# bdaiinstitute/judo

Measured on AMD Instinct MI355X. Metric: rollouts/sec + plan-step ms, leap_cube MPPI 65536xH64, higher is better.
Workload: dtype f32

## Files before the change

### judo_amd/csrc/jh_engine_v5.hip

```cpp
#include <cstddef>
#include <type_traits>

#include "jh_coop.h"

using namespace jh_eng;
using namespace jh_coop;

namespace {

#ifdef JH_V5_WAVESTAMP
__device__ unsigned long long* g_wavestamp = nullptr;
__device__ int g_wavestamp_cap = 0;
#endif

constexpr int G = 16, RPW = 4, WAVE = 64;
constexpr int NCH = 4, NLK = 4;

constexpr int LSMAX = 16;
constexpr int WAVES_PER_EU = 2;
constexpr int WAVES_PER_BLOCK = 4;
constexpr int BFS = 33;
constexpr int PAS = 9;
constexpr int RSPAD = 4;
constexpr int C3PAD = 278;
constexpr int NSLDS = 3;
constexpr double BIGPROB = 0.999999;
constexpr int CVX_STOP_NM = 1000;
#define OPAQUE(x) asm volatile("" : "+v"(x))
#define WSYNC() do { __builtin_amdgcn_fence(__ATOMIC_RELEASE, "wavefront"); __builtin_amdgcn_wave_barrier(); __builtin_amdgcn_fence(__ATOMIC_ACQUIRE, "wavefront"); } while (0)
#ifndef JH_V5_NSLOT
#define JH_V5_NSLOT 2
#endif
#ifndef JH_V5_NSBIG
#define JH_V5_NSBIG 3
#endif
#ifndef JH_V5_CYL
#define JH_V5_CYL 0
#endif
constexpr int GCYL = 5;
constexpr int NSLOT = JH_V5_NSLOT;
constexpr int NSBIG = JH_V5_NSBIG;
constexpr int NCP = 16 * (NSBIG < NSLDS ? NSBIG : NSLDS);
constexpr int NCAP = 16 * NSBIG;
constexpr int NOVF = NCAP - NCP;
constexpr int MAXHIT = 64;
constexpr int POOL_F = 10;
constexpr int MAXG = 80, MAXLG = 8;
constexpr int CUBE = 17;
constexpr int HITPAIR = 1 << 15;
static_assert(MAXG <= 128, "hand geom pairs are packed into 14 bits");
constexpr int MAXBP = 128;
constexpr int PT_SLOT = JH_PT_SLOT, PT_MAX = JH_PT_MAX, PT_I = JH_PT_I;
constexpr int MAXBPL = 96;
constexpr int NDH = 22 * 23 / 2;
constexpr int NV = 22, NQ = 23, NU = 16, NS = 31, NS_CALTECH = 23, NX = 45, NMB = 17;
constexpr int NBC = 20;
__device__ __forceinline__ bool static_code(int b) { return b == 0 || b >= NMB; }

enum { LC_DAMP = 0, LC_KVD, LC_KP, LC_KV, LC_CLO, LC_CHI, LC_CLIM, LC_FL, LC_FB, LC_FD, LC_INVW, LC_LIMITED, LC_LO, LC_HI, LC_LK, LC_LB, LC_SI, LC_IMCK = LC_SI + 5, LC_N = 25 };

struct __attribute__((aligned(16))) RS {
  float pa[NMB][PAS];
  float xR[NMB][9];
  float qv[NV], g[NV], p[NV], ws[NV];
  float acn[6];
  float Mbb[NCH][10];
  float rhs6[6];
  float cmd[4];
  union {
    struct {
      float bs[NBC][4];
      unsigned short hits[MAXHIT];
      unsigned char bpl[MAXBPL];
    };
    struct { float pk_q[G], pk_fs[G], pk_cq[4], pk_acc; };
  };
  union {
    float pool[NCP][POOL_F];
    struct { float Hcc[21], Hbb[NCH][10], Hcb[NCH][24], Hx[6][16]; };
    struct { float Hd[NDH], dinv[NV]; };
    struct { float c3pad_[C3PAD]; float c3s[G][12]; };
  };
  int ncon, nhit;
  float pad_[RSPAD];
};

static_assert(offsetof(RS, c3s) % 16 == 0 && C3PAD >= NDH + NV && sizeof(((RS*)nullptr)->c3pad_) + sizeof(((RS*)nullptr)->c3s) <= sizeof(((RS*)nullptr)->pool), "c3 cache: aligned rows behind the Newton matrices, inside the pool's storage");
struct PoolCtx { RS* S; int* overflow; float* ovf; };

__device__ __forceinline__ void push_contact(const PoolCtx& pc, const float* pos, const float* n, float dist, int body, float mu, float tran) {
  int i = atomicAdd(&pc.S->ncon, 1);
  float* e;
  if (i < NCP) e = pc.S->pool[i];
  else if (NOVF > 0 && pc.ovf && i < NCAP) e = pc.ovf + (i - NCP) * POOL_F;
  else { if (pc.overflow) atomicAdd(pc.overflow, 1); return; }
  e[0] = pos[0]; e[1] = pos[1]; e[2] = pos[2]; e[3] = n[0]; e[4] = n[1]; e[5] = n[2]; e[6] = dist; e[7] = mu; e[8] = __int_as_float(body); e[9] = tran;
}

struct LeapSink {
  PoolCtx pc; int sides; float mu, tran; bool flip;
  __device__ __forceinline__ void push(const float* pos, const float* n, float dist) {
// ... 822 lines not shown
    if (lc[LC_LIMITED] != 0.f) {
      float dlo = q - lc[LC_LO], dhi = lc[LC_HI] - q, dist = fminf(dlo, dhi);
      if (dist < 0.f) {
        float sg = dlo < dhi ? 1.f : -1.f, imp = impedance(lc + LC_SI, dist), R = fmaxf(1e-15f, (1.f - imp) / imp * lc[LC_INVW]);
        dr.lims = sg; dr.lD = 1.f / R; dr.laref = -lc[LC_LB] * (sg * qd) - lc[LC_LK] * imp * dist;
      }
    }
    bool anyslot = false; int cmask = 0; unsigned used = 0;
#pragma unroll
    for (int k = 0; k < NS; k++) {
      anyslot |= sl[k].la >= 0;
      used |= __any(sl[k].la >= 0) ? 1u << k : 0u;
      if (HC && sl[k].la > 0 && sl[k].la != CUBE && sl[k].lb > 0 && ((sl[k].la - 1) >> 2) != ((sl[k].lb - 1) >> 2)) cmask |= 1 << (4 * ((sl[k].la - 1) >> 2) + ((sl[k].lb - 1) >> 2));
    }
    int lvl = 0, par = -1, nlev = 0; bool dense_row = false;
    if constexpr (HC) {
      cmask = gor(cmask);
      if (__any(cmask != 0)) dense_row = !chain_elim_order(cmask, c, lvl, par, nlev);
#ifdef JH_V5_COUNT
      if (l == 0 && live) {
        int dmax = 0;
        for (int a = 0; a < NCH; a++) { int d = 0; for (int b = 0; b < NCH; b++) if (b != a) d += (cmask >> (a < b ? 4 * a + b : 4 * b + a)) & 1; dmax = d > dmax ? d : dmax; }
        cnt_cls[cmask == 0 ? 0 : (dense_row ? 3 : (dmax <= 1 ? 1 : 2))]++;
      }
#endif
    }
    S.pk_q[l] = q; S.pk_fs[l] = fs_own;
    if (l == 0) { S.pk_cq[0] = qc[3]; S.pk_cq[1] = qc[4]; S.pk_cq[2] = qc[5]; S.pk_cq[3] = qc[6]; S.pk_acc = acc; }
    const float Mdiag_own = sel4(Mrow, s), iMd = 1.f / Mdiag_own;
    const float fsc_own = mck * a0c_own;
    const float snorm = gsum(fs_own * fs_own * iMd + fsc_own * fsc_own * lc[LC_IMCK]);
    const bool has_rows = gor((int)(anyslot || dr.fl > 0.f || dr.lims != 0.f)) != 0;
    iters_this = 0;
    if (!has_rows) { a_own = a0_own; ac_own = a0c_own; }
    else {
      {
        const float qws = S.ws[6 + l];
        float xl[3] = {S.ws[0], S.ws[1], S.ws[2]}, xr[3] = {S.ws[3], S.ws[4], S.ws[5]}, wa[3]; mulMV(wa, S.xR[0], xr);
        const float wsc_own = l < 3 ? S.ws[l] : (l == 3 ? wa[0] : (l == 4 ? wa[1] : (l == 5 ? wa[2] : 0.f)));
        float cs = 0.f, jx[3], jar_ws[NS][3];
#pragma unroll
        for (int k = 0; k < NS; k++) if (sl[k].la >= 0) {
          slot_Jx<HC>(sl[k], S, qc, xl, wa, S.ws, jx, V5_C3C(k));
          for (int rw = 0; rw < 3; rw++) { sl[k].jar[rw] = jx[rw] - sl[k].aref[rw]; jar_ws[k][rw] = sl[k].jar[rw]; }
          cs += cone_cost(sl[k]);
        }
        const float jf_ws = qws - dr.faref, jl_ws = dr.lims * qws - dr.laref;
        dr.jf = jf_ws; dr.jl = jl_ws;
        cs += dof_rows_cost(dr);
        float dws = qws - a0_own, md = 0.f;
#pragma unroll
        for (int j = 0; j < NLK; j++) md += Mrow[j] * (quad_get(qws, j) - quad_get(a0_own, j));
        cs += 0.5f * dws * md;
        { float dcw = wsc_own - a0c_own; cs += 0.5f * dcw * dcw * mck; }
        const float cost_ws = gsum(cs);
        S.p[6 + l] = a0_own; if (l < 6) S.p[l] = a0c_own;
        WSYNC();
        float xl0[3] = {S.p[0], S.p[1], S.p[2]}, xr0[3] = {S.p[3], S.p[4], S.p[5]};
        wa[0] = xr0[0]; wa[1] = xr0[1]; wa[2] = xr0[2];
        cs = 0.f;
#pragma unroll
        for (int k = 0; k < NS; k++) if (sl[k].la >= 0) {
          slot_Jx<HC>(sl[k], S, qc, xl0, wa, S.p, jx, V5_C3C(k));
          for (int rw = 0; rw < 3; rw++) sl[k].jar[rw] = jx[rw] - sl[k].aref[rw];
          cs += cone_cost(sl[k]);
        }
        dr.jf = a0_own - dr.faref; dr.jl = dr.lims * a0_own - dr.laref;
        cs += dof_rows_cost(dr);
        const float cost_0 = gsum(cs);
        if (cost_ws < cost_0) {
          a_own = qws; ac_own = wsc_own;
#pragma unroll
          for (int k = 0; k < NS; k++) if (sl[k].la >= 0) for (int rw = 0; rw < 3; rw++) sl[k].jar[rw] = jar_ws[k][rw];
          dr.jf = jf_ws; dr.jl = jl_ws;
        } else { a_own = a0_own; ac_own = a0c_own; }
        WSYNC();
      }
      bool act = true;
      V5_TICK(3)
      auto forget_slots = [&]() __attribute__((always_inline)) {
#pragma unroll
        for (int k = 0; k < NS; k++) { OPAQUE(sl[k].la); OPAQUE(sl[k].lb); OPAQUE(sl[k].rc[0]); OPAQUE(sl[k].rc[1]); OPAQUE(sl[k].rc[2]); }
      };
      auto newton_loop = [&](auto dense_tag) __attribute__((always_inline)) {
      constexpr bool DENSE = decltype(dense_tag)::value;
      for (int it = 0; it < cap && __any(act); it++) {
        forget_slots();
        const float da_own = a_own - a0_own, dcl = ac_own - a0c_own;
        float g_own = 0.f, hd = 0.f;
#pragma unroll
        for (int j = 0; j < NLK; j++) g_own += Mrow[j] * quad_get(da_own, j);
        {
          const float D = dr.fD, x = dr.jf, fl = dr.fl, lim = dr.fR * fl;
          const bool has = fl > 0.f, lo_ = x <= -lim, hi_ = x >= lim, mid = has & !lo_ & !hi_;
          float ga = g_own - fl, gb = g_own + fl, gm = fmaf(D, x, g_own); asm volatile("" : "+v"(ga), "+v"(gb), "+v"(gm));
          g_own = has ? (lo_ ? ga : (hi_ ? gb : gm)) : g_own;
          hd = mid ? hd + D : hd;
          const bool lon = (dr.lims != 0.f) & (dr.jl < 0.f);
          g_own = lon ? fmaf(dr.lims * dr.lD, dr.jl, g_own) : g_own;
          hd = lon ? hd + dr.lD : hd;
        }
        S.g[6 + l] = g_own;
        const bool aact0 = act && !(DENSE && dense_row);
        {
          float* hb = &S.Hbb[c][tri(s, 0)];
#pragma unroll
          for (int j = 0; j < NLK; j++) hb[j < s ? j : s] = j < s ? Mrow[j] : Mdiag_own + hd;
          for (int k = 0; k < 6; k++) S.Hcb[c][s * 6 + k] = 0.f;
          if (HC) for (int k = 0; k < 6; k++) S.Hx[0][l * 6 + k] = 0.f;
        }
        float hcp[21];
#pragma unroll
        for (int e = 0; e < 21; e++) hcp[e] = 0.f;
        bool hcany = false;
        WSYNC();
        float gcp[6] = {0, 0, 0, 0, 0, 0};
        {
#pragma unroll
          for (int k = 0; k < NS; k++) {
            if (k > 0 && !((used >> k) & 1u)) continue;
            const Slot& t = sl[k];
            float f[3], Wk[6];
            const float D[3] = {t.D0, t.D1, t.D1};
            ConeZ cz;
            if (cone_top(t.jar, t.mu, t.fri, cz) | !act) continue;
            cone_below(t.jar, D, t.Dm, t.mu, t.fri, cz, f, Wk);
            bool on = true;
            if constexpr (DENSE) on = aact0;
            const float Fw[3] = {t.fr[0] * f[0] + t.fr[3] * f[1] + t.fr[6] * f[2], t.fr[1] * f[0] + t.fr[4] * f[1] + t.fr[7] * f[2], t.fr[2] * f[0] + t.fr[5] * f[1] + t.fr[8] * f[2]};
            const float pos[3] = {t.rc[0] + qc[0], t.rc[1] + qc[1], t.rc[2] + qc[2]};
            const bool cube = !HC || t.la == CUBE;
            float A[6];
            if (on) {
              float T0[3], T1[3], T2[3];
#pragma unroll
              for (int q = 0; q < 3; q++) {
                T0[q] = Wk[0] * t.fr[q] + Wk[1] * t.fr[3 + q] + Wk[3] * t.fr[6 + q];
                T1[q] = Wk[1] * t.fr[q] + Wk[2] * t.fr[3 + q] + Wk[4] * t.fr[6 + q];
                T2[q] = Wk[3] * t.fr[q] + Wk[4] * t.fr[3 + q] + Wk[5] * t.fr[6 + q];
              }
#pragma unroll
              for (int i = 0; i < 3; i++)
#pragma unroll
                for (int j = 0; j <= i; j++) A[tri(i, j)] = t.fr[i] * T0[j] + t.fr[3 + i] * T1[j] + t.fr[6 + i] * T2[j];
            }
            auto Amul = [&](const float* v, float* y) __attribute__((always_inline)) {
              y[0] = A[0] * v[0] + A[1] * v[1] + A[3] * v[2]; y[1] = A[1] * v[0] + A[2] * v[1] + A[4] * v[2]; y[2] = A[3] * v[0] + A[4] * v[1] + A[5] * v[2];
            };
            if (cube) {
              float tb[3]; cross3(tb, t.rc, Fw);
              gcp[0] += Fw[0]; gcp[1] += Fw[1]; gcp[2] += Fw[2]; gcp[3] += tb[0]; gcp[4] += tb[1]; gcp[5] += tb[2];
              if (on) {
#pragma unroll
                for (int e = 0; e < 6; e++) hcp[e] += A[e];
                const float rx = t.rc[0], ry = t.rc[1], rz = t.rc[2];
                const float Ac[3][3] = {{A[0], A[1], A[3]}, {A[1], A[2], A[4]}, {A[3], A[4], A[5]}};
                float zq[3][3];
#pragma unroll
                for (int i = 0; i < 3; i++) { zq[0][i] = ry * Ac[2][i] - rz * Ac[1][i]; zq[1][i] = rz * Ac[0][i] - rx * Ac[2][i]; zq[2][i] = rx * Ac[1][i] - ry * Ac[0][i]; }
#pragma unroll
                for (int q = 0; q < 3; q++) {
#pragma unroll
                  for (int r2 = 0; r2 < 3; r2++) hcp[tri(3 + q, r2)] += zq[q][r2];
                }
                hcp[tri(3, 3)] += ry * zq[0][2] - rz * zq[0][1];
                hcp[tri(4, 3)] += ry * zq[1][2] - rz * zq[1][1]; hcp[tri(4, 4)] += rz * zq[1][0] - rx * zq[1][2];
                hcp[tri(5, 3)] += ry * zq[2][2] - rz * zq[2][1]; hcp[tri(5, 4)] += rz * zq[2][0] - rx * zq[2][2]; hcp[tri(5, 5)] += rx * zq[2][1] - ry * zq[2][0];
                hcany = true;
              }
            }
            if (t.lb > 0) {
              const int ch = (t.lb - 1) >> 2, dep = (t.lb - 1) & 3;
              const bool linkA = HC && !cube && t.la > 0;
              const int cha = linkA ? (t.la - 1) >> 2 : 0, depa = linkA ? (t.la - 1) & 3 : -1;
              const bool same = linkA && cha == ch;
              float cb[NLK][3]; if (V5_C3C(k)) load_c3(V5_C3C(k), cb); else link_c3(S, ch, pos, cb);
              if constexpr (!HC) {
#pragma unroll
                for (int u4 = 0; u4 < NLK; u4++) if (u4 <= dep) {
                  atomicAdd(&S.g[6 + 4 * ch + u4], -dot3(cb[u4], Fw));
                  float y[3]; Amul(cb[u4], y);
#pragma unroll
                  for (int v4 = 0; v4 <= u4; v4++) atomicAdd(&S.Hbb[ch][tri(u4, v4)], dot3(cb[v4], y));
#pragma unroll
                  for (int q = 0; q < 3; q++) atomicAdd(&S.Hcb[ch][u4 * 6 + q], -y[q]);
                  atomicAdd(&S.Hcb[ch][u4 * 6 + 3], t.rc[2] * y[1] - t.rc[1] * y[2]);
                  atomicAdd(&S.Hcb[ch][u4 * 6 + 4], t.rc[0] * y[2] - t.rc[2] * y[0]);
                  atomicAdd(&S.Hcb[ch][u4 * 6 + 5], t.rc[1] * y[0] - t.rc[0] * y[1]);
                }
              } else {
              float fjs[NLK];
#pragma unroll
              for (int u4 = 0; u4 < NLK; u4++) {
                fjs[u4] = dot3(cb[u4], Fw);
                const float sg = (u4 <= dep ? 1.f : 0.f) - ((same && u4 <= depa) ? 1.f : 0.f);
                cb[u4][0] *= sg; cb[u4][1] *= sg; cb[u4][2] *= sg;
                if (u4 <= dep) {
                  atomicAdd(&S.g[6 + 4 * ch + u4], -fjs[u4]);
                  if (on) {
                    float y[3]; Amul(cb[u4], y);
#pragma unroll
                    for (int v4 = 0; v4 <= u4; v4++) atomicAdd(&S.Hbb[ch][tri(u4, v4)], dot3(cb[v4], y));
                    const float hv[6] = {-y[0], -y[1], -y[2], t.rc[2] * y[1] - t.rc[1] * y[2], t.rc[0] * y[2] - t.rc[2] * y[0], t.rc[1] * y[0] - t.rc[0] * y[1]};
                    if (cube) {
#pragma unroll
                      for (int q = 0; q < 6; q++) atomicAdd(&S.Hcb[ch][u4 * 6 + q], hv[q]);
                    }
                  }
                }
              }
              if (__any(same)) {
#pragma unroll
                for (int j = 0; j < NLK; j++) if (same && j <= depa) atomicAdd(&S.g[6 + 4 * ch + j], fjs[j]);
              }
              if (linkA && !same) {
                float ca[NLK][3]; link_c3(S, cha, pos, ca);
#pragma unroll
                for (int j = 0; j < NLK; j++) {
                  if (j <= depa) atomicAdd(&S.g[6 + 4 * cha + j], dot3(ca[j], Fw));
                  const float sg = j <= depa ? 1.f : 0.f;
                  ca[j][0] *= sg; ca[j][1] *= sg; ca[j][2] *= sg;
                }
                if (on) {
#pragma unroll
                  for (int u4 = 0; u4 < NLK; u4++) if (u4 <= depa) {
                    float y[3]; Amul(ca[u4], y);
#pragma unroll
                    for (int v4 = 0; v4 <= u4; v4++) atomicAdd(&S.Hbb[cha][tri(u4, v4)], dot3(ca[v4], y));
#pragma unroll
                    for (int v4 = 0; v4 < NLK; v4++) if (v4 <= dep) atomicAdd(&S.Hx[pidx(cha, ch)][v4 * 4 + u4], -dot3(cb[v4], y));
                  }
                }
              }
              }
            }
          }
        }
        float gcl = 0.f;
        float h0 = 0.f, h1;
        {
          const float v2[16] = {hcp[16], hcp[17], hcp[18], hcp[19], hcp[20], 0.f, 0.f, 0.f, gcp[0], gcp[1], gcp[2], gcp[3], gcp[4], gcp[5], 0.f, 0.f};
          h1 = row_scatter16(v2, l);
          const float gq = dppf<0x128>(h1);
          gcl = l < 6 ? gq : 0.f;
          if (__any(hcany)) h0 = row_scatter16(hcp, l);
        }
        gcl = fmaf(mck, dcl, gcl);
        {
          constexpr int HCC_G = ((int)offsetof(RS, Hcc) - (int)offsetof(RS, g)) / 4 - 6;
          float* gl = &S.g[6 + l];
          gl[HCC_G] = h0;
          if (l < 5) gl[HCC_G + 16] = h1;
        }
        WSYNC();
        V5_TICK(4)
        g_own = S.g[6 + l];
        const float gn = gsum(g_own * g_own * iMd + gcl * gcl * lc[LC_IMCK]);
        act = act & !(gn <= tol * tol * fmaxf(snorm, 1e-12f));
        if (!__any(act)) break;
        iters_this += act ? 1 : 0;
        n_wave_iters++;
        const bool aact = act && !(DENSE && dense_row);
        V5_TICK(5)
        float L[10], Linv[4], Ya[NLK], Yb[NLK], zb[NLK], xc6[6], pc4[NLK];
        const bool hasb = s < 2;
        auto factor_block = [&]() __attribute__((always_inline)) {
          for (int k = 0; k < 10; k++) L[k] = S.Hbb[c][k];
          chol4(L, Linv);
          for (int j = 0; j < NLK; j++) { Ya[j] = S.Hcb[c][j * 6 + s]; const float yb = (&S.Hcb[0][0])[c * 24 + j * 6 + 4 + (s & 1)]; Yb[j] = hasb ? yb : 0.f; }
          fwd4(L, Linv, Ya); fwd4(L, Linv, Yb);
          asm volatile("" : "+v"(Yb[0]), "+v"(Yb[1]), "+v"(Yb[2]), "+v"(Yb[3]));
          for (int j = 0; j < NLK; j++) zb[j] = -S.g[6 + 4 * c + j];
          fwd4(L, Linv, zb);
        };
        factor_block();
        if (l < 6) S.rhs6[l] = -gcl;
        float Xs[NLK] = {0.f, 0.f, 0.f, 0.f};
        if constexpr (HC) {
#pragma unroll 1
          for (int st = 1; st < NCH; st++) {
            if (!__any(aact && nlev >= st)) break;
            const bool me = aact && lvl == st - 1 && par >= 0;
            if (me) {
              const float* hx = par > c ? S.Hx[pidx(c, par)] : S.Hx[pidx(par, c)];
              for (int j = 0; j < NLK; j++) Xs[j] = par > c ? hx[s * 4 + j] : hx[j * 4 + s];
              fwd4(L, Linv, Xs);
            }
#pragma unroll
            for (int j = 0; j < NLK; j++) {
              const float v = Xs[0] * quad_get(Xs[0], j) + Xs[1] * quad_get(Xs[1], j) + Xs[2] * quad_get(Xs[2], j) + Xs[3] * quad_get(Xs[3], j);
              if (me && j <= s) atomicAdd(&S.Hbb[par][tri(s, j)], -v);
            }
#pragma unroll
            for (int q6 = 0; q6 < 6; q6++) {
              float v = 0.f;
#pragma unroll
              for (int j = 0; j < NLK; j++) v += Xs[j] * (q6 < 4 ? quad_get(Ya[j], q6) : quad_get(Yb[j], q6 - 4));
              if (me) atomicAdd(&S.Hcb[par][s * 6 + q6], -v);
            }
            if (me) atomicAdd(&S.g[6 + 4 * par + s], Xs[0] * zb[0] + Xs[1] * zb[1] + Xs[2] * zb[2] + Xs[3] * zb[3]);
            WSYNC();
            if (lvl == st) factor_block();
          }
        }
        WSYNC();
        V5_TICK(6)
        {
          float dar[6], dbr[6];
#pragma unroll
          for (int r6 = 0; r6 < 6; r6++) {
            float Yr[NLK];
#pragma unroll
            for (int j = 0; j < NLK; j++) Yr[j] = r6 < 4 ? quad_get(Ya[j], r6) : quad_get(Yb[j], r6 - 4);
            float da = Ya[0] * Yr[0] + Ya[1] * Yr[1] + Ya[2] * Yr[2] + Ya[3] * Yr[3], db = Yb[0] * Yr[0] + Yb[1] * Yr[1] + Yb[2] * Yr[2] + Yb[3] * Yr[3];
            dar[r6] = qsum4_same(da); dbr[r6] = qsum4_same(db);
            continue;
            da = qsum4(da); db = qsum4(db);
            const bool app = aact && c == 0;
            if (app) {
              if (r6 <= s) atomicAdd(&S.Hcc[tri(s, r6)], -da);
              if (hasb && r6 <= 4 + s) atomicAdd(&S.Hcc[tri(4 + s, r6)], -db);
            }
          }
          float ra = Ya[0] * zb[0] + Ya[1] * zb[1] + Ya[2] * zb[2] + Ya[3] * zb[3], rb = Yb[0] * zb[0] + Yb[1] * zb[1] + Yb[2] * zb[2] + Yb[3] * zb[3];
          ra = qsum4_same(ra); rb = qsum4_same(rb);
          float Lc[21];
#pragma unroll
          for (int q6 = 0; q6 < 6; q6++) {
#pragma unroll
            for (int r6 = 0; r6 <= q6; r6++) Lc[tri(q6, r6)] = (r6 == q6 ? S.Hcc[tri(q6, r6)] + S.cmd[q6 < 3 ? 0 : q6 - 2] : S.Hcc[tri(q6, r6)]) - (q6 < 4 ? quad_get(dar[r6], q6) : quad_get(dbr[r6], q6 - 4));
            xc6[q6] = S.rhs6[q6] - (q6 < 4 ? quad_get(ra, q6) : quad_get(rb, q6 - 4));
          }
          float ci[6];
#pragma unroll
          for (int i = 0; i < 6; i++)
#pragma unroll
            for (int j = 0; j <= i; j++) {
              float sv = Lc[tri(i, j)];
#pragma unroll
              for (int k = 0; k < j; k++) sv -= Lc[tri(i, k)] * Lc[tri(j, k)];
              if (i == j) { float rr = __frsqrt_rn(fmaxf(sv, 1e-30f)); ci[i] = rr; Lc[tri(i, i)] = sv * rr; }
              else Lc[tri(i, j)] = sv * ci[j];
            }
#pragma unroll
          for (int i = 0; i < 6; i++) { float sv = xc6[i];
#pragma unroll
            for (int k = 0; k < i; k++) sv -= Lc[tri(i, k)] * xc6[k];
            xc6[i] = sv * ci[i]; }
#pragma unroll
          for (int i = 5; i >= 0; i--) { float sv = xc6[i];
#pragma unroll
            for (int k = i + 1; k < 6; k++) sv -= Lc[tri(k, i)] * xc6[k];
            xc6[i] = sv * ci[i]; }
          asm volatile("" : "+v"(xc6[0]), "+v"(xc6[1]), "+v"(xc6[2]), "+v"(xc6[3]), "+v"(xc6[4]), "+v"(xc6[5]));
          float xa = sel4o(xc6, s), xb = s == 0 ? xc6[4] : xc6[5]; asm volatile("" : "+v"(xb));
#pragma unroll
          for (int j = 0; j < NLK; j++) pc4[j] = zb[j] - csum(fmaf(Ya[j], xa, Yb[j] * xb));
          if constexpr (HC) {
            if (__any(aact && nlev > 0)) {
#pragma unroll 1
              for (int st = NCH - 1; st >= 0; st--) {
                if (!__any(aact && nlev >= st)) continue;
                const bool me = aact && lvl == st;
                const float pbs = (me && par >= 0) ? S.p[6 + 4 * par + s] : 0.f;
#pragma unroll
                for (int j = 0; j < NLK; j++) pc4[j] -= csum(Xs[j] * pbs);
                if (st > 0) {
                  float pb4[NLK];
                  for (int j = 0; j < NLK; j++) pb4[j] = pc4[j];
                  bwd4(L, Linv, pb4);
                  if (me) S.p[6 + l] = sel4(pb4, s);
                  WSYNC();
                }
              }
            }
          }
          bwd4(L, Linv, pc4);
        }
        asm volatile("" : "+v"(pc4[0]), "+v"(pc4[1]), "+v"(pc4[2]), "+v"(pc4[3]));
        float p_own = sel4o(pc4, s);
        float xcl;
        { float x03 = sel4o(xc6, l & 3), x45 = (l & 1) ? xc6[5] : xc6[4]; asm volatile("" : "+v"(x45)); xcl = l < 4 ? x03 : (l < 6 ? x45 : 0.f); asm volatile("" : "+v"(xcl)); }
        S.p[6 + l] = p_own; if (l < 6) S.p[l] = xcl;
        WSYNC();
        if constexpr (HC && DENSE) {
#ifdef JH_V5_COUNT
        if (lane == 0) { cnt_it++; cnt_dense += __any(act && dense_row) ? 1 : 0; }
#endif
        if (__any(act && dense_row)) {
          const bool dact = act && dense_row;
          if (dact) for (int e = l; e < NDH; e += G) S.Hd[e] = 0.f;
          WSYNC();
          if (dact) {
#pragma unroll
            for (int j = 0; j < NLK; j++) if (j <= s) S.Hd[tri(6 + l, 6 + 4 * c + j)] = Mrow[j] + (j == s ? hd : 0.f);
            if (l < 6) { S.Hd[tri(l, l)] = mck; S.g[l] = gcl; }
          }
          WSYNC();
#pragma unroll
          for (int k = 0; k < NS; k++) {
            const Slot& t = sl[k];
            if (!(dact && t.la >= 0)) continue;
            float f[3], Wk[6];
            const float D[3] = {t.D0, t.D1, t.D1};
            cone_eval(t.jar, D, t.Dm, t.mu, t.fri, f, Wk);
            if (Wk[0] == 0.f && Wk[2] == 0.f && Wk[5] == 0.f) continue;
            const float pos[3] = {t.rc[0] + qc[0], t.rc[1] + qc[1], t.rc[2] + qc[2]};
            float X0[6][3], X1[NLK][3];
            for (int j = 0; j < 6; j++) X0[j][0] = X0[j][1] = X0[j][2] = 0.f;
            for (int j = 0; j < NLK; j++) X1[j][0] = X1[j][1] = X1[j][2] = 0.f;
            int o0 = 0, n0 = 0, o1 = 0, n1 = 0;
            if (t.la == CUBE) {
              n0 = 6;
              for (int q3 = 0; q3 < 3; q3++) {
                X0[q3][0] = -t.fr[q3]; X0[q3][1] = -t.fr[3 + q3]; X0[q3][2] = -t.fr[6 + q3];
                const float ea[3] = {q3 == 0 ? 1.f : 0.f, q3 == 1 ? 1.f : 0.f, q3 == 2 ? 1.f : 0.f}; float c3[3]; cross3(c3, ea, t.rc);
                X0[3 + q3][0] = -dot3(t.fr, c3); X0[3 + q3][1] = -dot3(t.fr + 3, c3); X0[3 + q3][2] = -dot3(t.fr + 6, c3);
              }
            } else if (t.la > 0) { o0 = 6 + 4 * ((t.la - 1) >> 2); n0 = 1 + ((t.la - 1) & 3); link_cols(S, t.la, pos, t.fr, -1.f, X0); }
            if (t.lb > 0) {
              o1 = 6 + 4 * ((t.lb - 1) >> 2); n1 = 1 + ((t.lb - 1) & 3);
              if (t.la != CUBE && t.la > 0 && o1 == o0) { link_cols(S, t.lb, pos, t.fr, 1.f, X0); n0 = n0 > n1 ? n0 : n1; n1 = 0; }
              else link_cols(S, t.lb, pos, t.fr, 1.f, X1);
            }
            if (n1 > 0 && n0 > 0 && o1 < o0) {
              for (int j = 0; j < NLK; j++) for (int q = 0; q < 3; q++) { const float tmp = X0[j][q]; X0[j][q] = X1[j][q]; X1[j][q] = tmp; }
              int ti = o0; o0 = o1; o1 = ti; ti = n0; n0 = n1; n1 = ti;
            }
#pragma unroll
            for (int u = 0; u < 6; u++) if (u < n0) {
              const float* j3 = X0[u];
              const float G0 = Wk[0] * j3[0] + Wk[1] * j3[1] + Wk[3] * j3[2], G1 = Wk[1] * j3[0] + Wk[2] * j3[1] + Wk[4] * j3[2], G2 = Wk[3] * j3[0] + Wk[4] * j3[1] + Wk[5] * j3[2];
#pragma unroll
              for (int v = 0; v <= u; v++) atomicAdd(&S.Hd[tri(o0 + u, o0 + v)], X0[v][0] * G0 + X0[v][1] * G1 + X0[v][2] * G2);
#pragma unroll
              for (int v = 0; v < NLK; v++) if (v < n1) atomicAdd(&S.Hd[tri(o1 + v, o0 + u)], X1[v][0] * G0 + X1[v][1] * G1 + X1[v][2] * G2);
            }
#pragma unroll
            for (int u = 0; u < NLK; u++) if (u < n1) {
              const float* j3 = X1[u];
              const float G0 = Wk[0] * j3[0] + Wk[1] * j3[1] + Wk[3] * j3[2], G1 = Wk[1] * j3[0] + Wk[2] * j3[1] + Wk[4] * j3[2], G2 = Wk[3] * j3[0] + Wk[4] * j3[1] + Wk[5] * j3[2];
#pragma unroll
              for (int v = 0; v <= u; v++) atomicAdd(&S.Hd[tri(o1 + u, o1 + v)], X1[v][0] * G0 + X1[v][1] * G1 + X1[v][2] * G2);
            }
          }
          WSYNC();
          const int r1 = 16 + l;
          const bool two = l < 6;
          float h0[16], h1[NV];
#pragma unroll
          for (int j = 0; j < 16; j++) h0[j] = (dact && j <= l) ? S.Hd[tri(l, j)] : 0.f;
#pragma unroll
          for (int j = 0; j < NV; j++) h1[j] = (dact && two && j <= r1) ? S.Hd[tri(r1, j)] : 0.f;
#pragma unroll
          for (int kk = 0; kk < NV; kk++) {
            float dp = 0.f, s0 = kk < 16 ? h0[kk < 16 ? kk : 0] : 0.f, s1 = h1[kk];
            const float hkk = dact ? S.Hd[tri(kk, kk)] : 1.f;
#pragma unroll
            for (int j = 0; j < kk; j++) {
              const float t = dact ? S.Hd[tri(kk, j)] : 0.f;
              dp = fmaf(t, t, dp);
              if (kk < 16) s0 = fmaf(-h0[j < 16 ? j : 0], t, s0);
              s1 = fmaf(-h1[j], t, s1);
            }
            const float rk = __frsqrt_rn(fmaxf(hkk - dp, 1e-30f));
            if (kk < 16) h0[kk < 16 ? kk : 0] = kk <= l ? s0 * rk : 0.f;
            h1[kk] = (two && kk <= r1) ? s1 * rk : 0.f;
            if (dact) {
              if (kk < 16 && l > kk) S.Hd[tri(l, kk)] = h0[kk < 16 ? kk : 0];
              if (two && r1 > kk) S.Hd[tri(r1, kk)] = h1[kk];
              if (l == 0) S.dinv[kk] = rk;
            }
            WSYNC();
          }
          float b0 = dact ? -S.g[l] : 0.f, b1 = (dact && two) ? -S.g[r1] : 0.f;
#pragma unroll
          for (int kk = 0; kk < NV; kk++) {
            if (dact && (kk < 16 ? l == kk : r1 == kk)) S.p[kk] = (kk < 16 ? b0 : b1) * S.dinv[kk];
            WSYNC();
            const float yk = dact ? S.p[kk] : 0.f;
            if (kk < 16) b0 -= (l > kk ? h0[kk < 16 ? kk : 0] : 0.f) * yk;
            b1 -= ((two && r1 > kk) ? h1[kk] : 0.f) * yk;
          }
#pragma unroll
          for (int kk = NV - 1; kk >= 0; kk--) {
            if (dact && (kk < 16 ? l == kk : r1 == kk)) {
              const float xk = S.p[kk] * S.dinv[kk];
              S.p[kk] = xk;
#pragma unroll
              for (int j = 0; j < kk; j++) S.p[j] -= (kk < 16 ? h0[j < 16 ? j : 0] : h1[j]) * xk;
            }
            WSYNC();
          }
          if (dact) {
            p_own = S.p[6 + l]; xcl = l < 6 ? S.p[l] : 0.f;
            for (int k = 0; k < 6; k++) xc6[k] = S.p[k];
            for (int j = 0; j < NLK; j++) pc4[j] = S.p[6 + 4 * c + j];
          }
        }
}
        V5_TICK(9)
        float Mp_own = 0.f;
#pragma unroll
        for (int j = 0; j < NLK; j++) Mp_own += Mrow[j] * pc4[j];
        const float pMp = gsum(p_own * Mp_own + mck * xcl * xcl);
        const float pMd = gsum(Mp_own * da_own + mck * xcl * dcl);
        const float gp = gsum(g_own * p_own + gcl * xcl);
        if (act && !(gp < 0.f)) act = false;
        {
          const float* wa = xc6 + 3;
#pragma unroll
          for (int k = 0; k < NS; k++) {
            if (!HC && k == 0) { slot_Jx_first(sl[0], xc6, wa, S.p, sl[0].jp, V5_C3C(0)); continue; }
            if (k > 0 && !((used >> k) & 1u)) continue;
            if (sl[k].la >= 0) slot_Jx<HC>(sl[k], S, qc, xc6, wa, S.p, sl[k].jp, V5_C3C(k));
          }
        }
        dr.pf = p_own; dr.pl = dr.lims * p_own;
        V5_TICK(10)
        float lo = 0.f, hi = -1.f, alpha = 1.f; bool lsact = act;
#ifdef JH_V5_CENSUS
        int cen_ls = 0, cen_lsw = 0; const bool cen_act = act;
        if (stats && lane == 0) atomicAdd(stats + 320 + __popcll(__ballot(act && l == 0)), 1);
#endif
        for (int ls = 0; ls < LSMAX && __any(lsact); ls++) {
          float d1, d2;
#ifdef JH_V5_CENSUS
          cen_ls += lsact; cen_lsw++;
#endif
          lane_rows_dir<NS>(sl, dr, alpha, &d1, &d2, used);
          d1 = gsum(d1) + pMd + alpha * pMp; d2 = gsum(d2) + pMp;
          {
            const bool upd = lsact & !(fabsf(d1) <= lstol * fabsf(gp)), neg = d1 < 0.f;
            lo = (upd & neg) ? alpha : lo; hi = (upd & !neg) ? alpha : hi;
            float nx = alpha - d1 * __builtin_amdgcn_rcpf(d2);
            const bool out_lo = nx <= lo, out_hi = nx >= hi;
            float dbl = 2.f * alpha, mid_ = 0.5f * (lo + hi); asm volatile("" : "+v"(dbl), "+v"(mid_));
            nx = hi < 0.f ? (out_lo ? dbl : nx) : ((out_lo | out_hi) ? mid_ : nx);
            alpha = upd ? nx : alpha; lsact = upd;
          }
        }
#ifdef JH_V5_CENSUS
        if (stats) { if (l == 0 && live && cen_act) atomicAdd(stats + 256 + min(cen_ls, 31), 1); if (lane == 0) atomicAdd(stats + 288 + min(cen_lsw, 31), 1); }
#endif
        V5_TICK(11)
        if (act) {
          a_own += alpha * p_own; ac_own += alpha * xcl;
#pragma unroll
          for (int k = 0; k < NS; k++) if (sl[k].la >= 0) for (int rw = 0; rw < 3; rw++) sl[k].jar[rw] += alpha * sl[k].jp[rw];
          dr.jf += alpha * dr.pf; dr.jl += alpha * dr.pl;
          if (-gp * alpha <= tol * tol * fmaxf(snorm, 1e-12f)) act = false;
        }
        WSYNC();
        V5_TICK(12)
      }
      };
      if constexpr (HC && NS > NSLOT) newton_loop(std::true_type{});
      else if constexpr (HC && NS == NSLOT) { if (__any(dense_row)) newton_loop(std::true_type{}); else newton_loop(std::false_type{}); }
      else newton_loop(std::false_type{});
      if (l == 0) { n_iters += iters_this; n_maxed += (iters_this >= cap); }
    }
    };
    if (__builtin_expect_with_probability(NSBIG > NSLOT && __any(S.ncon > 16 * NSLOT), 0, BIGPROB)) {
      if (NOVF > 0 && __any(S.ncon > NCP)) __threadfence();
      solve_step(std::integral_constant<int, NSBIG>{}, std::integral_constant<bool, SELF>{});
    } else {
      if (SELF && !__any(hand_hits)) solve_step(std::integral_constant<int, NSLOT>{}, std::false_type{});
      else solve_step(std::integral_constant<int, NSLOT>{}, std::integral_constant<bool, SELF>{});
    }
#ifdef JH_V5_CENSUS
    if (stats) { if (l == 0 && live) atomicAdd(stats + 192 + min(iters_this, 31), 1); if (lane == 0) atomicAdd(stats + 224 + min(n_wave_iters - wave_it0, 31), 1); }
#endif
    {
      S.ws[6 + l] = a_own; if (l < 6) { S.acn[l] = ac_own; if (l < 3) S.ws[l] = ac_own; }
      q = S.pk_q[l]; qd = S.qv[6 + l]; fs_own = S.pk_fs[l];
      const float da_own = a_own - a0_own;
      float rhs_own = fs_own, x4[NLK], L[10];
#pragma unroll
      for (int j = 0; j < NLK; j++) rhs_own += Mrow[j] * quad_get(da_own, j);
#pragma unroll
      for (int j = 0; j < NLK; j++) x4[j] = quad_get(rhs_own, j);
      for (int k = 0; k < 10; k++) L[k] = S.Mbb[c][k];
      const float hdk = h * (lc[LC_DAMP] + lc[LC_KVD]);
#pragma unroll
      for (int j = 0; j < NLK; j++) L[tri(j, j)] += quad_get(hdk, j);
      float inv4[4]; chol4(L, inv4); fwd4(L, inv4, x4); bwd4(L, inv4, x4);
      const float qacc = sel4(x4, s);
      qd = fmaf(h, qacc, qd); q = fmaf(h, qd, q);
      WSYNC();
      for (int k = 0; k < 6; k++) vc[k] = S.qv[k];
      for (int k = 0; k < 4; k++) qc[3 + k] = S.pk_cq[k];
      if (!MATERIALIZE) acc = S.pk_acc;
      {
        const float aw[3] = {S.acn[3], S.acn[4], S.acn[5]}; float ab[3]; mulMTV(ab, S.xR[0], aw);
        for (int k = 0; k < 3; k++) { vc[k] = fmaf(h, S.acn[k], vc[k]); vc[3 + k] = fmaf(h, ab[k], vc[3 + k]); }
        if (l < 3) S.ws[3 + l] = l == 0 ? ab[0] : (l == 1 ? ab[1] : ab[2]);
      }
      for (int k = 0; k < 3; k++) qc[k] = fmaf(h, vc[k], qc[k]);
      float wn = sqrtf(vc[3] * vc[3] + vc[4] * vc[4] + vc[5] * vc[5]), ang = wn * h;
      if (ang > 0.f) {
        float sn, cs; sincosf(0.5f * ang, &sn, &cs); float kk = sn / wn;
        float dq[4] = {cs, vc[3] * kk, vc[4] * kk, vc[5] * kk}, *qq = qc + 3;
        float r0 = qq[0] * dq[0] - qq[1] * dq[1] - qq[2] * dq[2] - qq[3] * dq[3];
        float r1 = qq[0] * dq[1] + qq[1] * dq[0] + qq[2] * dq[3] - qq[3] * dq[2];
        float r2 = qq[0] * dq[2] - qq[1] * dq[3] + qq[2] * dq[0] + qq[3] * dq[1];
        float r3 = qq[0] * dq[3] + qq[1] * dq[2] - qq[2] * dq[1] + qq[3] * dq[0];
        qq[0] = r0; qq[1] = r1; qq[2] = r2; qq[3] = r3;
      }
      float nn = rsqrtf(qc[3] * qc[3] + qc[4] * qc[4] + qc[5] * qc[5] + qc[6] * qc[6]);
      qc[3] *= nn; qc[4] *= nn; qc[5] *= nn; qc[6] *= nn;
    }
    V5_TICK(7)
    if (MATERIALIZE) {
      if (states && live) {
        float* o = states + ((size_t)nc * H + hh) * NX;
        o[7 + l] = q; o[NQ + 6 + l] = qd;
        if (l < 7) o[l] = qc[l];
        if (l < 6) o[NQ + l] = vc[l];
      }
    } else acc += leap_step_cost(sTp, qc);
    WSYNC();
  }
#ifdef JH_V5_COUNT
  if (stats) { if (lane == 0) { atomicAdd(stats + 24, cnt_dense); atomicAdd(stats + 25, cnt_it); atomicAdd(stats + 26, cnt_l2); atomicAdd(stats + 28, H); } if (l == 0 && live) { atomicAdd(stats + 27, cnt_bp); atomicAdd(stats + 29, cnt_hh); for (int k = 0; k < 4; k++) atomicAdd(stats + 30 + k, cnt_cls[k]); } }
#endif
#ifdef JH_V5_TICKS
  if (lane == 0 && stats) { for (int k = 0; k < 8; k++) atomicAdd((unsigned long long*)(stats + 4) + k, (unsigned long long)cyc[k]);
                            for (int k = 0; k < 16; k++) atomicAdd((unsigned long long*)(stats + 384) + k, (unsigned long long)cyc[k]); }
#endif
  if (!MATERIALIZE && live && l == 0) costs[n] = acc / (float)H;
  if (stats && live && l == 0) { if (n_maxed) atomicAdd(stats + 1, n_maxed); atomicAdd(stats + 2, n_iters); atomicAdd(stats + 3, H); }
  if (stats && lane == 0 && live) { atomicAdd(stats + 20, n_wave_iters); atomicAdd(stats + 21, H); }
#ifdef JH_V5_WAVESTAMP
  if (lane == 0 && g_wavestamp && grp < g_wavestamp_cap) {
    unsigned long long* w = g_wavestamp + (size_t)grp * 6;
    w[0] = ((unsigned long long)blockIdx.x << 32) | ((unsigned long long)wv << 8) | (__smid() & 0xff); w[1] = ws_entry; w[2] = ws_staged; w[3] = ws_start; w[4] = wall_clock64(); w[5] = 1;
  }
#endif
  if constexpr (!PERSIST) break;
  else {
    int t = 0;
    if (lane == 0) t = (int)atomicAdd(head, 1u);
// ... 91 lines not shown
```

Before: 1.286 million.

## Add gradient-only convergence check and drop hand-contact path when hand rows finish

Adds two changes to the Newton solver loop. First, once the previous step's decrease falls below a kappa multiple of the tolerance, the next iteration runs a gradient-only contact pass, with no Hessian assembly, and exits early if every row has converged. This avoids a full Hessian build and factorisation on the last iteration. Second, in the NSLOT hand-contact specialisation, once no active row has hand contacts, the loop leaves and resumes in a cheaper variant without the hand-contact (HC) code paths. Both add code size and register pressure, and each gradient-only check costs an extra contact pass when it fails to terminate.

```diff
diff --git a/judo_amd/csrc/jh_engine_v5.hip b/judo_amd/csrc/jh_engine_v5.hip
--- a/judo_amd/csrc/jh_engine_v5.hip
+++ b/judo_amd/csrc/jh_engine_v5.hip
@@ -17,6 +17,16 @@
 constexpr int NCH = 4, NLK = 4;
 
 constexpr int LSMAX = 16;
+#ifndef JH_V5_KAPPA
+#define JH_V5_KAPPA 64.f
+#endif
+#ifndef JH_V5_PIECE_A
+#define JH_V5_PIECE_A 1
+#endif
+#ifndef JH_V5_PIECE_B
+#define JH_V5_PIECE_B 1
+#endif
+constexpr float NEWTON_END_KAPPA = JH_V5_KAPPA;
 constexpr int WAVES_PER_EU = 2;
 constexpr int WAVES_PER_BLOCK = 4;
 constexpr int BFS = 33;
@@ -1005,12 +1015,27 @@
 #pragma unroll
         for (int k = 0; k < NS; k++) { OPAQUE(sl[k].la); OPAQUE(sl[k].lb); OPAQUE(sl[k].rc[0]); OPAQUE(sl[k].rc[1]); OPAQUE(sl[k].rc[2]); }
       };
-      auto newton_loop = [&](auto dense_tag) __attribute__((always_inline)) {
+      int it = 0;
+#ifdef JH_V5_COUNT
+      int cnt_bin = 0;
+#endif
+      bool ending = false;
+      const unsigned long long hand_rows = __ballot(hand_hits);
+      auto newton_loop = [&](auto dense_tag, auto hc_tag, auto leave_tag) __attribute__((always_inline)) {
       constexpr bool DENSE = decltype(dense_tag)::value;
-      for (int it = 0; it < cap && __any(act); it++) {
+      constexpr bool HCL = decltype(hc_tag)::value;
+      constexpr bool LEAVE = decltype(leave_tag)::value;
+      for (; it < cap && __any(act) && !(LEAVE && (__ballot(act) & hand_rows) == 0ull); it++) {
         forget_slots();
         const float da_own = a_own - a0_own, dcl = ac_own - a0c_own;
-        float g_own = 0.f, hd = 0.f;
+        float g_own, hd, gcl;
+#ifdef JH_V5_COUNT
+        const int cnt_wbin = it == 0 ? 32 : wave_rowmax(act ? cnt_bin : -1);
+        if (lane == 0) { V5_CADD(490, 1); V5_CADD(491, HC && NS == NSLOT); V5_CADD(492, HC && NS == NSLOT && (__ballot(act) & hand_rows) == 0ull); }
+#endif
+        auto contact_pass = [&](auto hess_tag) __attribute__((always_inline)) {
+        constexpr bool HESS = decltype(hess_tag)::value;
+        g_own = 0.f; hd = 0.f;
 #pragma unroll
         for (int j = 0; j < NLK; j++) g_own += Mrow[j] * quad_get(da_own, j);
         {
@@ -1025,12 +1050,12 @@
         }
         S.g[6 + l] = g_own;
         const bool aact0 = act && !(DENSE && dense_row);
-        {
+        if constexpr (HESS) {
           float* hb = &S.Hbb[c][tri(s, 0)];
 #pragma unroll
           for (int j = 0; j < NLK; j++) hb[j < s ? j : s] = j < s ? Mrow[j] : Mdiag_own + hd;
           for (int k = 0; k < 6; k++) S.Hcb[c][s * 6 + k] = 0.f;
-          if (HC) for (int k = 0; k < 6; k++) S.Hx[0][l * 6 + k] = 0.f;
+          if (HCL) for (int k = 0; k < 6; k++) S.Hx[0][l * 6 + k] = 0.f;
         }
         float hcp[21];
 #pragma unroll
@@ -1048,11 +1073,11 @@
             ConeZ cz;
             if (cone_top(t.jar, t.mu, t.fri, cz) | !act) continue;
             cone_below(t.jar, D, t.Dm, t.mu, t.fri, cz, f, Wk);
-            bool on = true;
-            if constexpr (DENSE) on = aact0;
+            bool on = HESS;
+            if constexpr (HESS && DENSE) on = aact0;
             const float Fw[3] = {t.fr[0] * f[0] + t.fr[3] * f[1] + t.fr[6] * f[2], t.fr[1] * f[0] + t.fr[4] * f[1] + t.fr[7] * f[2], t.fr[2] * f[0] + t.fr[5] * f[1] + t.fr[8] * f[2]};
             const float pos[3] = {t.rc[0] + qc[0], t.rc[1] + qc[1], t.rc[2] + qc[2]};
-            const bool cube = !HC || t.la == CUBE;
+            const bool cube = !HCL || t.la == CUBE;
             float A[6];
             if (on) {
               float T0[3], T1[3], T2[3];
@@ -1094,14 +1119,15 @@
             }
             if (t.lb > 0) {
               const int ch = (t.lb - 1) >> 2, dep = (t.lb - 1) & 3;
-              const bool linkA = HC && !cube && t.la > 0;
+              const bool linkA = HCL && !cube && t.la > 0;
               const int cha = linkA ? (t.la - 1) >> 2 : 0, depa = linkA ? (t.la - 1) & 3 : -1;
               const bool same = linkA && cha == ch;
               float cb[NLK][3]; if (V5_C3C(k)) load_c3(V5_C3C(k), cb); else link_c3(S, ch, pos, cb);
-              if constexpr (!HC) {
+              if constexpr (!HCL) {
 #pragma unroll
                 for (int u4 = 0; u4 < NLK; u4++) if (u4 <= dep) {
                   atomicAdd(&S.g[6 + 4 * ch + u4], -dot3(cb[u4], Fw));
+                  if constexpr (HESS) {
                   float y[3]; Amul(cb[u4], y);
 #pragma unroll
                   for (int v4 = 0; v4 <= u4; v4++) atomicAdd(&S.Hbb[ch][tri(u4, v4)], dot3(cb[v4], y));
@@ -1110,6 +1136,7 @@
                   atomicAdd(&S.Hcb[ch][u4 * 6 + 3], t.rc[2] * y[1] - t.rc[1] * y[2]);
                   atomicAdd(&S.Hcb[ch][u4 * 6 + 4], t.rc[0] * y[2] - t.rc[2] * y[0]);
                   atomicAdd(&S.Hcb[ch][u4 * 6 + 5], t.rc[1] * y[0] - t.rc[0] * y[1]);
+                  }
                 }
               } else {
               float fjs[NLK];
@@ -1159,7 +1186,7 @@
             }
           }
         }
-        float gcl = 0.f;
+        gcl = 0.f;
         float h0 = 0.f, h1;
         {
           const float v2[16] = {hcp[16], hcp[17], hcp[18], hcp[19], hcp[20], 0.f, 0.f, 0.f, gcp[0], gcp[1], gcp[2], gcp[3], gcp[4], gcp[5], 0.f, 0.f};
@@ -1169,17 +1196,39 @@
           if (__any(hcany)) h0 = row_scatter16(hcp, l);
         }
         gcl = fmaf(mck, dcl, gcl);
-        {
+        if constexpr (HESS) {
           constexpr int HCC_G = ((int)offsetof(RS, Hcc) - (int)offsetof(RS, g)) / 4 - 6;
           float* gl = &S.g[6 + l];
           gl[HCC_G] = h0;
           if (l < 5) gl[HCC_G + 16] = h1;
         }
         WSYNC();
+        };
+        if (JH_V5_PIECE_A && ending) {
+          contact_pass(std::false_type{});
+          V5_TICK(15)
+#ifdef JH_V5_TICKS
+          if (lane == 0 && stats) atomicAdd(stats + 416, 1);
+#endif
+          const float g1 = S.g[6 + l];
+          const float gn1 = gsum(g1 * g1 * iMd + gcl * gcl * lc[LC_IMCK]);
+          const bool all_done = !__any(act & !(gn1 <= tol * tol * fmaxf(snorm, 1e-12f)));
+#ifdef JH_V5_COUNT
+          if (lane == 0) { V5_CADD(all_done ? 488 : 489, 1); if (all_done) V5_CADD(420 + 2 * cnt_wbin + 1, 1); }
+#endif
+          if (all_done) { act = false; break; }
+        }
+        contact_pass(std::true_type{});
         V5_TICK(4)
+#ifdef JH_V5_TICKS
+        if (lane == 0 && stats) atomicAdd(stats + 417, 1);
+#endif
         g_own = S.g[6 + l];
         const float gn = gsum(g_own * g_own * iMd + gcl * gcl * lc[LC_IMCK]);
         act = act & !(gn <= tol * tol * fmaxf(snorm, 1e-12f));
+#ifdef JH_V5_COUNT
+        if (lane == 0) V5_CADD(420 + 2 * cnt_wbin + (__any(act) ? 0 : 1), 1);
+#endif
         if (!__any(act)) break;
         iters_this += act ? 1 : 0;
         n_wave_iters++;
@@ -1199,7 +1248,7 @@
         factor_block();
         if (l < 6) S.rhs6[l] = -gcl;
         float Xs[NLK] = {0.f, 0.f, 0.f, 0.f};
-        if constexpr (HC) {
+        if constexpr (HCL) {
 #pragma unroll 1
           for (int st = 1; st < NCH; st++) {
             if (!__any(aact && nlev >= st)) break;
@@ -1279,7 +1328,7 @@
           float xa = sel4o(xc6, s), xb = s == 0 ? xc6[4] : xc6[5]; asm volatile("" : "+v"(xb));
 #pragma unroll
           for (int j = 0; j < NLK; j++) pc4[j] = zb[j] - csum(fmaf(Ya[j], xa, Yb[j] * xb));
-          if constexpr (HC) {
+          if constexpr (HCL) {
             if (__any(aact && nlev > 0)) {
 #pragma unroll 1
               for (int st = NCH - 1; st >= 0; st--) {
@@ -1306,7 +1355,7 @@
         { float x03 = sel4o(xc6, l & 3), x45 = (l & 1) ? xc6[5] : xc6[4]; asm volatile("" : "+v"(x45)); xcl = l < 4 ? x03 : (l < 6 ? x45 : 0.f); asm volatile("" : "+v"(xcl)); }
         S.p[6 + l] = p_own; if (l < 6) S.p[l] = xcl;
         WSYNC();
-        if constexpr (HC && DENSE) {
+        if constexpr (HCL && DENSE) {
 #ifdef JH_V5_COUNT
         if (lane == 0) { cnt_it++; cnt_dense += __any(act && dense_row) ? 1 : 0; }
 #endif
@@ -1434,9 +1483,9 @@
           const float* wa = xc6 + 3;
 #pragma unroll
           for (int k = 0; k < NS; k++) {
-            if (!HC && k == 0) { slot_Jx_first(sl[0], xc6, wa, S.p, sl[0].jp, V5_C3C(0)); continue; }
+            if (!HCL && k == 0) { slot_Jx_first(sl[0], xc6, wa, S.p, sl[0].jp, V5_C3C(0)); continue; }
             if (k > 0 && !((used >> k) & 1u)) continue;
-            if (sl[k].la >= 0) slot_Jx<HC>(sl[k], S, qc, xc6, wa, S.p, sl[k].jp, V5_C3C(k));
+            if (sl[k].la >= 0) slot_Jx<HCL>(sl[k], S, qc, xc6, wa, S.p, sl[k].jp, V5_C3C(k));
           }
         }
         dr.pf = p_own; dr.pl = dr.lims * p_own;
@@ -1474,13 +1523,26 @@
           dr.jf += alpha * dr.pf; dr.jl += alpha * dr.pl;
           if (-gp * alpha <= tol * tol * fmaxf(snorm, 1e-12f)) act = false;
         }
+        ending = !__any(act && !(-gp * alpha <= NEWTON_END_KAPPA * (tol * tol * fmaxf(snorm, 1e-12f))));
+#ifdef JH_V5_COUNT
+        cnt_bin = min(max((int)floorf(2.f * log2f(-gp * alpha / (tol * tol * fmaxf(snorm, 1e-12f)))), 0), 31);
+#endif
         WSYNC();
         V5_TICK(12)
       }
       };
-      if constexpr (HC && NS > NSLOT) newton_loop(std::true_type{});
-      else if constexpr (HC && NS == NSLOT) { if (__any(dense_row)) newton_loop(std::true_type{}); else newton_loop(std::false_type{}); }
-      else newton_loop(std::false_type{});
+      if constexpr (HC && NS > NSLOT) newton_loop(std::true_type{}, std::true_type{}, std::false_type{});
+      else if constexpr (HC && NS == NSLOT) {
+        constexpr bool LEAVE = JH_V5_PIECE_B != 0;
+        if (__any(dense_row)) newton_loop(std::true_type{}, std::true_type{}, std::integral_constant<bool, LEAVE>{});
+        else newton_loop(std::false_type{}, std::true_type{}, std::integral_constant<bool, LEAVE>{});
+#ifdef JH_V5_COUNT
+        if (LEAVE && it < cap && __any(act) && lane == 0) V5_CADD(493, 1);
+#endif
+        if (LEAVE && it < cap && __any(act))
+          newton_loop(std::false_type{}, std::false_type{}, std::false_type{});
+      }
+      else newton_loop(std::false_type{}, std::false_type{}, std::false_type{});
       if (l == 0) { n_iters += iters_this; n_maxed += (iters_this >= cap); }
     }
     };
```

Result: no change. 1.290 million (median of 6 runs) (+0.3%).
